# dazzmo/ik

Hardware: NVIDIA B200
Metric: converged IK solves/sec (Cassie, batch 65,536) (higher is better)
Workload: dtype f64

## Files before the change

### ik_b200/csrc/spec_cassie_feet_pelvis.cu

```cuda
#include <cstdlib>
#include <cstring>

#include "dls_spec.cuh"
#include "dls_team.cuh"
#include "gen/cassie_feet_pelvis.cuh"
#include "gen/cassie_feet_pelvis_arrow.cuh"
#include "gen/cassie_feet_pelvis_arrow_b.cuh"
#include "gen/cassie_feet_pelvis_w1.cuh"
#include "gen/cassie_feet_pelvis_w2.cuh"

namespace ikb {
namespace {
using S3 = SpecCassieFeetPelvis;
using SA = SpecCassieFeetPelvisArrow;
using S2 = SpecCassieFeetPelvisW2;
using S1 = SpecCassieFeetPelvisW1;
using SB = SpecCassieFeetPelvisArrowB;
int solve_variant(bool f64, bool tail) {
    const char *e = std::getenv("IKB_CASSIE_SOLVE");
    if (e && std::strcmp(e, "dense") == 0) return 0;
    if (e && std::strcmp(e, "arrow") == 0) return 1;
    if (e && std::strcmp(e, "arrowb") == 0) return 2;
    return (f64 && !tail) ? 1 : 2;
}
int roles(int dflt) {
    const char *e = std::getenv("IKB_CASSIE_ROLES");
    return (e && e[0] >= '1' && e[0] <= '3') ? e[0] - '0' : dflt;
}

struct TeamTree {
    bool ok = false;
    int chain[2][kTeamChain];
    TeamTree() {
        if (S3::NJOINTS != 18 || S3::NTASKS != 3 || S3::NQ != 23 || S3::M != 12) return;
        const int *par = S3::sig_parent(), *typ = S3::sig_type(), *tj = S3::sig_task_joint(), *tt = S3::sig_task_type();
        if (tj[0] != 1 || typ[1] != IKB_J_FREEFLYER || tt[0] != IKB_FULL || tt[1] != IKB_POSITION || tt[2] != IKB_POSITION) return;
        const double *fp = S3::sig_task_placement();
        for (int i = 0; i < 12; ++i)
            if (fp[i] != ((i == 0 || i == 4 || i == 8) ? 1.0 : 0.0)) return;
        for (int l = 0; l < 2; ++l) {
            int j = tj[1 + l], n = 0, rev[32];
            while (j > 1 && n < 32) {
                rev[n++] = j;
                j = par[j];
            }
            if (j != 1 || n != kTeamChain) return;
            for (int k = 0; k < kTeamChain; ++k) {
                chain[l][k] = rev[kTeamChain - 1 - k];
                if (typ[chain[l][k]] != IKB_J_RZ || chain[l][k] != 2 + 8 * l + (k < 6 ? k : 7)) return;
            }
        }
        ok = true;
    }
};
const TeamTree &team_tree() {
    static const TeamTree t;
    return t;
}
template <typename T> TeamConsts<T> team_consts(const SpecHostConsts &hc) {
    TeamConsts<T> c{};
    const TeamTree &t = team_tree();
    const double *pl = S3::sig_placement(), *fp = S3::sig_task_placement();
    for (int l = 0; l < 2; ++l) {
        for (int k = 0; k < kTeamChain; ++k) {
            const double *p = pl + 15 * t.chain[l][k];
            for (int i = 0; i < 9; ++i) c.PR[l][k][i] = (T)p[i];
            for (int i = 0; i < 3; ++i) c.Pp[l][k][i] = (T)p[9 + i];
        }
        for (int i = 0; i < 9; ++i) c.FR[l][i] = (T)fp[12 * (1 + l) + i];
        for (int i = 0; i < 3; ++i) c.Fp[l][i] = (T)fp[12 * (1 + l) + 9 + i];
    }
    for (int k = 0; k < S3::NQ; ++k) {
        c.lower[k] = (T)hc.lower[k];
        c.upper[k] = (T)hc.upper[k];
    }
    for (int i = 0; i < S3::M; ++i) c.weight[i] = (T)hc.weight[i];
    return c;
}
bool use_team(bool is_f64, bool resume) {
    const char *e = std::getenv("IKB_CASSIE_TAIL");
    if (!team_tree().ok || (e && e[0] == '0')) return false;
    if (e && e[0] == 't') return true;
    return !(is_f64 && resume);
}

template <typename T> int launch(const SpecHostConsts &hc, const SolveArgs<T> &a, int variant, long long n, int sms, cudaStream_t s,
                                 int bulk_roles) {
    if (variant == SPEC_TAIL) {
        if (use_team(sizeof(T) == 8, a.resume != 0)) return launch_team<T>(team_consts<T>(hc), a, n, sms, s);
        switch (solve_variant(sizeof(T) == 8, true)) {
            case 0: return launch_spec_tail<S3, T>(hc, a, n, sms, s);
            case 1: return launch_spec_tail<SA, T>(hc, a, n, sms, s);
            default: return launch_spec_tail<SB, T>(hc, a, n, sms, s);
        }
    }
    switch (roles(bulk_roles)) {
        case 3:
            switch (solve_variant(sizeof(T) == 8, false)) {
                case 0: return launch_spec_bulk<S3, T>(hc, a, n, sms, s);
                case 1: return launch_spec_bulk<SA, T>(hc, a, n, sms, s);
                default: return launch_spec_bulk<SB, T>(hc, a, n, sms, s);
            }
        case 2: return launch_spec_bulk<S2, T>(hc, a, n, sms, s);
        default: return launch_spec_bulk<S1, T>(hc, a, n, sms, s);
    }
}
int l64(const SpecHostConsts &hc, const SolveArgs<double> &a, int v, long long n, int sms, cudaStream_t s) {
    return launch<double>(hc, a, v, n, sms, s, 3);
}
int l32(const SpecHostConsts &hc, const SolveArgs<float> &a, int v, long long n, int sms, cudaStream_t s) {
    return launch<float>(hc, a, v, n, sms, s, 3);
}
}
extern const SpecializedKernel kSpecCassieFeetPelvis = {S3::name(), spec_matches<S3>, l64, l32, spec_near_miss<S3>};
}
```

### ik_b200/csrc/spec_common.hpp

```cpp
#pragma once
#include "se3_math.cuh"

#define IKB_PHASE_FENCE() asm volatile("" ::: "memory")

namespace ikb {

template <typename T, int NQ, int M> struct SpecConsts {
    T lower[NQ], upper[NQ];
    T weight[M];
    T mask[M];
};

template <typename T, int STRIDE> struct Strip {
    static constexpr int kStride = STRIDE;
    T *base;
    IKB_HD void set(int k, T v) const { base[k * STRIDE] = v; }
    IKB_HD T get(int k) const { return base[k * STRIDE]; }
    IKB_HD T operator[](int k) const { return base[k * STRIDE]; }
    IKB_HD void flush() const {}
    IKB_HD void copy_in(int k, const T *src) const {
#if defined(__CUDA_ARCH__)
        static_assert(sizeof(T) == 4 || sizeof(T) == 8, "cp.async copies 4, 8 or 16 bytes");
        const unsigned dst = (unsigned)__cvta_generic_to_shared(base + k * STRIDE);
        if (sizeof(T) == 8)
            asm volatile("cp.async.ca.shared.global [%0], [%1], 8;" ::"r"(dst), "l"(src) : "memory");
        else
            asm volatile("cp.async.ca.shared.global [%0], [%1], 4;" ::"r"(dst), "l"(src) : "memory");
#else
        base[k * STRIDE] = *src;
#endif
    }
};
IKB_HD void strip_copies_wait() {
#if defined(__CUDA_ARCH__)
    asm volatile("cp.async.wait_all;" ::: "memory");
#endif
}

}
```

### ik_b200/csrc/tmem_scratch.cuh

```cuda
#pragma once
#include <cstdint>

namespace ikb {

template <int COLS> __device__ __forceinline__ uint32_t tmem_provision(uint32_t *slot, int warp) {
    static_assert(COLS == 32 || COLS == 64 || COLS == 128 || COLS == 256 || COLS == 512, "TMEM allocations are powers of two >= 32 columns");
    if (warp == 0) {
        const uint32_t dst = (uint32_t)__cvta_generic_to_shared(slot);
        asm volatile("tcgen05.alloc.cta_group::1.sync.aligned.shared::cta.b32 [%0], %1;" ::"r"(dst), "r"((uint32_t)COLS) : "memory");
        asm volatile("tcgen05.relinquish_alloc_permit.cta_group::1.sync.aligned;" ::: "memory");
    }
    asm volatile("tcgen05.fence::before_thread_sync;" ::: "memory");
    __syncthreads();
    asm volatile("tcgen05.fence::after_thread_sync;" ::: "memory");
    const uint32_t base = *reinterpret_cast<volatile uint32_t *>(slot);
    __syncthreads();
    return base;
}
template <int COLS> __device__ __forceinline__ void tmem_release(uint32_t base, int warp) {
    asm volatile("tcgen05.fence::before_thread_sync;" ::: "memory");
    __syncthreads();
    if (warp == 0) asm volatile("tcgen05.dealloc.cta_group::1.sync.aligned.b32 %0, %1;" ::"r"(base), "r"((uint32_t)COLS) : "memory");
}

__device__ __forceinline__ void tmem_ld32(uint32_t addr, uint32_t (&r)[32]) {
    asm volatile(
        "tcgen05.ld.sync.aligned.32x32b.x32.b32 {%0, %1, %2, %3, %4, %5, %6, %7, %8, %9, %10, %11, %12, %13, %14, %15, %16, %17, %18, %19, "
        "%20, %21, %22, %23, %24, %25, %26, %27, %28, %29, %30, %31}, [%32];"
        : "=r"(r[0]), "=r"(r[1]), "=r"(r[2]), "=r"(r[3]), "=r"(r[4]), "=r"(r[5]), "=r"(r[6]), "=r"(r[7]), "=r"(r[8]), "=r"(r[9]),
          "=r"(r[10]), "=r"(r[11]), "=r"(r[12]), "=r"(r[13]), "=r"(r[14]), "=r"(r[15]), "=r"(r[16]), "=r"(r[17]), "=r"(r[18]), "=r"(r[19]),
          "=r"(r[20]), "=r"(r[21]), "=r"(r[22]), "=r"(r[23]), "=r"(r[24]), "=r"(r[25]), "=r"(r[26]), "=r"(r[27]), "=r"(r[28]), "=r"(r[29]),
          "=r"(r[30]), "=r"(r[31])
        : "r"(addr)
        : "memory");
    asm volatile("tcgen05.wait::ld.sync.aligned;" ::: "memory");
}
__device__ __forceinline__ void tmem_st32(uint32_t addr, const uint32_t (&r)[32]) {
    asm volatile(
        "tcgen05.st.sync.aligned.32x32b.x32.b32 [%0], {%1, %2, %3, %4, %5, %6, %7, %8, %9, %10, %11, %12, %13, %14, %15, %16, %17, %18, %19, %20, "
        "%21, %22, %23, %24, %25, %26, %27, %28, %29, %30, %31, %32};"
        :
        : "r"(addr), "r"(r[0]), "r"(r[1]), "r"(r[2]), "r"(r[3]), "r"(r[4]), "r"(r[5]), "r"(r[6]), "r"(r[7]), "r"(r[8]), "r"(r[9]), "r"(r[10]),
          "r"(r[11]), "r"(r[12]), "r"(r[13]), "r"(r[14]), "r"(r[15]), "r"(r[16]), "r"(r[17]), "r"(r[18]), "r"(r[19]), "r"(r[20]), "r"(r[21]),
          "r"(r[22]), "r"(r[23]), "r"(r[24]), "r"(r[25]), "r"(r[26]), "r"(r[27]), "r"(r[28]), "r"(r[29]), "r"(r[30]), "r"(r[31])
        : "memory");
    asm volatile("tcgen05.wait::st.sync.aligned;" ::: "memory");
}

template <int N> __device__ __forceinline__ void tmem_park(uint32_t addr, const double (&v)[N]) {
    static_assert(N <= 16, "one x32 transfer carries 16 doubles");
    uint32_t r[32];
#pragma unroll
    for (int i = 0; i < 16; ++i) {
        r[2 * i] = i < N ? (uint32_t)__double2loint(v[i < N ? i : 0]) : 0u;
        r[2 * i + 1] = i < N ? (uint32_t)__double2hiint(v[i < N ? i : 0]) : 0u;
    }
    tmem_st32(addr, r);
}
template <int N> __device__ __forceinline__ void tmem_fetch(uint32_t addr, double (&v)[N]) {
    static_assert(N <= 16, "one x32 transfer carries 16 doubles");
    uint32_t r[32];
    tmem_ld32(addr, r);
#pragma unroll
    for (int i = 0; i < N; ++i) v[i] = __hiloint2double((int)r[2 * i + 1], (int)r[2 * i]);
}
template <typename T> struct TStrip {
    static_assert(sizeof(T) == 8, "tensor-memory strips hold doubles (two 32-bit columns per element)");
    static constexpr int kStride = 2;
    uint32_t base;
    __device__ __forceinline__ void set(int k, T v) const {
        asm volatile("tcgen05.st.sync.aligned.32x32b.x2.b32 [%0], {%1, %2};" ::"r"(base + (uint32_t)(k * 2)), "r"((uint32_t)__double2loint(v)),
                     "r"((uint32_t)__double2hiint(v))
                     : "memory");
    }
    __device__ __forceinline__ T get(int k) const {
        uint32_t lo, hi;
        asm volatile("tcgen05.ld.sync.aligned.32x32b.x2.b32 {%0, %1}, [%2];" : "=r"(lo), "=r"(hi) : "r"(base + (uint32_t)(k * 2)) : "memory");
        asm volatile("tcgen05.wait::ld.sync.aligned;" ::: "memory");
        return __hiloint2double((int)hi, (int)lo);
    }
    __device__ __forceinline__ void flush() const { asm volatile("tcgen05.wait::st.sync.aligned;" ::: "memory"); }
};

template <int N> __device__ __forceinline__ void tmem_park(uint32_t, const float (&)[N]) {}
template <int N> __device__ __forceinline__ void tmem_fetch(uint32_t, float (&)[N]) {}

}
```

Baseline: 192.6 million.

## Add folded Cassie arrow solve variant with batched TMEM strip loads

```diff
diff --git a/ik_b200/csrc/spec_cassie_feet_pelvis.cu b/ik_b200/csrc/spec_cassie_feet_pelvis.cu
--- a/ik_b200/csrc/spec_cassie_feet_pelvis.cu
+++ b/ik_b200/csrc/spec_cassie_feet_pelvis.cu
@@ -6,6 +6,7 @@
 #include "gen/cassie_feet_pelvis.cuh"
 #include "gen/cassie_feet_pelvis_arrow.cuh"
 #include "gen/cassie_feet_pelvis_arrow_b.cuh"
+#include "gen/cassie_feet_pelvis_fold.cuh"
 #include "gen/cassie_feet_pelvis_w1.cuh"
 #include "gen/cassie_feet_pelvis_w2.cuh"
 
@@ -16,12 +17,14 @@
 using S2 = SpecCassieFeetPelvisW2;
 using S1 = SpecCassieFeetPelvisW1;
 using SB = SpecCassieFeetPelvisArrowB;
+using SF = SpecCassieFeetPelvisFold;
 int solve_variant(bool f64, bool tail) {
     const char *e = std::getenv("IKB_CASSIE_SOLVE");
     if (e && std::strcmp(e, "dense") == 0) return 0;
     if (e && std::strcmp(e, "arrow") == 0) return 1;
     if (e && std::strcmp(e, "arrowb") == 0) return 2;
-    return (f64 && !tail) ? 1 : 2;
+    if (e && std::strcmp(e, "fold") == 0) return 3;
+    return (f64 && !tail) ? 3 : 2;
 }
 int roles(int dflt) {
     const char *e = std::getenv("IKB_CASSIE_ROLES");
@@ -91,6 +94,9 @@
         switch (solve_variant(sizeof(T) == 8, true)) {
             case 0: return launch_spec_tail<S3, T>(hc, a, n, sms, s);
             case 1: return launch_spec_tail<SA, T>(hc, a, n, sms, s);
+            case 3:
+                if constexpr (sizeof(T) == 8) return launch_spec_tail<SF, T>(hc, a, n, sms, s);
+                return launch_spec_tail<SB, T>(hc, a, n, sms, s);
             default: return launch_spec_tail<SB, T>(hc, a, n, sms, s);
         }
     }
@@ -99,6 +105,9 @@
             switch (solve_variant(sizeof(T) == 8, false)) {
                 case 0: return launch_spec_bulk<S3, T>(hc, a, n, sms, s);
                 case 1: return launch_spec_bulk<SA, T>(hc, a, n, sms, s);
+                case 3:
+                    if constexpr (sizeof(T) == 8) return a.nseg > 0 ? launch_spec_bulk<SF, T>(hc, a, n, sms, s) : launch_spec_bulk<SA, T>(hc, a, n, sms, s);
+                    return launch_spec_bulk<SB, T>(hc, a, n, sms, s);
                 default: return launch_spec_bulk<SB, T>(hc, a, n, sms, s);
             }
         case 2: return launch_spec_bulk<S2, T>(hc, a, n, sms, s);
diff --git a/ik_b200/csrc/spec_common.hpp b/ik_b200/csrc/spec_common.hpp
--- a/ik_b200/csrc/spec_common.hpp
+++ b/ik_b200/csrc/spec_common.hpp
@@ -17,6 +17,9 @@
     IKB_HD void set(int k, T v) const { base[k * STRIDE] = v; }
     IKB_HD T get(int k) const { return base[k * STRIDE]; }
     IKB_HD T operator[](int k) const { return base[k * STRIDE]; }
+    template <int N> IKB_HD void getn(int k, T (&v)[N]) const {
+        for (int i = 0; i < N; ++i) v[i] = base[(k + i) * STRIDE];
+    }
     IKB_HD void flush() const {}
     IKB_HD void copy_in(int k, const T *src) const {
 #if defined(__CUDA_ARCH__)
diff --git a/ik_b200/csrc/tmem_scratch.cuh b/ik_b200/csrc/tmem_scratch.cuh
--- a/ik_b200/csrc/tmem_scratch.cuh
+++ b/ik_b200/csrc/tmem_scratch.cuh
@@ -79,7 +79,54 @@
         asm volatile("tcgen05.wait::ld.sync.aligned;" ::: "memory");
         return __hiloint2double((int)hi, (int)lo);
     }
+    template <int N> __device__ __forceinline__ void getn(int k, T (&v)[N]) const {
+        uint32_t r[2 * N];
+        tmem_ld_run<2 * N>(base + (uint32_t)(k * 2), r);
+        asm volatile("tcgen05.wait::ld.sync.aligned;" ::: "memory");
+#pragma unroll
+        for (int i = 0; i < 2 * N; ++i) asm volatile("" : "+r"(r[i]));
+#pragma unroll
+        for (int i = 0; i < N; ++i) v[i] = __hiloint2double((int)r[2 * i + 1], (int)r[2 * i]);
+    }
     __device__ __forceinline__ void flush() const { asm volatile("tcgen05.wait::st.sync.aligned;" ::: "memory"); }
+
+  private:
+    template <int C> __device__ __forceinline__ static void ld_cols(uint32_t a, uint32_t *r) {
+        if constexpr (C == 16) {
+            asm volatile("tcgen05.ld.sync.aligned.32x32b.x16.b32 {%0, %1, %2, %3, %4, %5, %6, %7, %8, %9, %10, %11, %12, %13, %14, %15}, [%16];"
+                         : "=r"(r[0]), "=r"(r[1]), "=r"(r[2]), "=r"(r[3]), "=r"(r[4]), "=r"(r[5]), "=r"(r[6]), "=r"(r[7]), "=r"(r[8]),
+                           "=r"(r[9]), "=r"(r[10]), "=r"(r[11]), "=r"(r[12]), "=r"(r[13]), "=r"(r[14]), "=r"(r[15])
+                         : "r"(a)
+                         : "memory");
+        } else if constexpr (C == 8) {
+            asm volatile("tcgen05.ld.sync.aligned.32x32b.x8.b32 {%0, %1, %2, %3, %4, %5, %6, %7}, [%8];"
+                         : "=r"(r[0]), "=r"(r[1]), "=r"(r[2]), "=r"(r[3]), "=r"(r[4]), "=r"(r[5]), "=r"(r[6]), "=r"(r[7])
+                         : "r"(a)
+                         : "memory");
+        } else if constexpr (C == 4) {
+            asm volatile("tcgen05.ld.sync.aligned.32x32b.x4.b32 {%0, %1, %2, %3}, [%4];"
+                         : "=r"(r[0]), "=r"(r[1]), "=r"(r[2]), "=r"(r[3])
+                         : "r"(a)
+                         : "memory");
+        } else {
+            static_assert(C == 2, "runs are cut into 16, 8, 4 and 2 columns");
+            asm volatile("tcgen05.ld.sync.aligned.32x32b.x2.b32 {%0, %1}, [%2];" : "=r"(r[0]), "=r"(r[1]) : "r"(a) : "memory");
+        }
+    }
+    template <int NC> __device__ __forceinline__ static void tmem_ld_run(uint32_t a, uint32_t *r) {
+        if constexpr (NC >= 16) {
+            ld_cols<16>(a, r);
+            tmem_ld_run<NC - 16>(a + 16, r + 16);
+        } else if constexpr (NC >= 8) {
+            ld_cols<8>(a, r);
+            tmem_ld_run<NC - 8>(a + 8, r + 8);
+        } else if constexpr (NC >= 4) {
+            ld_cols<4>(a, r);
+            tmem_ld_run<NC - 4>(a + 4, r + 4);
+        } else if constexpr (NC >= 2) {
+            ld_cols<2>(a, r);
+        }
+    }
 };
 
 template <int N> __device__ __forceinline__ void tmem_park(uint32_t, const float (&)[N]) {}
```

Result: faster. 210.3 million (median of 6 runs) (+9.2%).
